# ShudaLi/rgbd_pose_estimation

Measured on AMD Instinct MI355X. Metric: correspondence-residuals/sec, higher is better.
Workload: dtype f32; 1 GPU; configs[1]: 640x480 dense depth, 307200 3D-3D corr, point-to-point GN step (K1 normal eq + host 6x6 solve + SE3 exp) over inlier mask; corr_rank0=307200, global_corr=307200, collective=none, rccl_ranks=0, rccl_verified=False, repeats=1

## Files before the change

### rgbd_pose_estimation_amd/csrc/rpe_host.hpp

```cpp
#pragma once
#include "../../include/rgbd_pose_hip.h"
#include "rpe_kernels.h"
#include "../include/rpe/linalg.hpp"

#include <dlfcn.h>
#include <rccl/rccl.h>

#include <cstdarg>
#include <ctime>
#include <cstdio>
#include <cstdlib>
#include <cmath>
#include <limits>
#include <atomic>
#include <chrono>
#include <condition_variable>
#include <mutex>
#include <string>
#include <vector>
#include <algorithm>
#include <cctype>
#include <sched.h>
#include <unistd.h>
#include <cstring>

struct rpe_context {
  int device = 0;
  hipStream_t stream = nullptr;
  struct { bool active = false; int kind = 0, mode = 0, grid = 0, runs = 0, batches = 0; double thre_3d = 0, cos_thr = 0, cos_nl = 0;
           unsigned long long base = 0, id = 0, slot_token = 0;
           double last_us = 0, wait_us = 2e6;
           bool pend_late = false;
           std::vector<double> seen_pose; std::vector<int> seen_votes;
           bool pending = false; unsigned long long pend_tag = 0; int pend_votes = 0; double pend_pose[7] = {0, 0, 0, 0, 0, 0, 0}; } sess;
  std::recursive_mutex sess_m;
  hipStream_t stream2 = nullptr;
// ... 261 lines not shown
inline rpe::PoseF pose_f(const double* p12) {
  rpe::PoseF T;
  for (int i = 0; i < 9; i++) T.R[i] = (float)p12[i];
  for (int i = 0; i < 3; i++) T.t[i] = (float)p12[9 + i];
  return T;
}
inline int ensure_maps(rpe_context* c, float** maps, int count, size_t* cap, int64_t n) {
  const size_t bytes = (size_t)n * 3 * sizeof(float);
  if (maps[0] && *cap >= bytes) return RPE_OK;
  HIP_TRY(hipStreamSynchronize(c->stream));
  for (int i = 0; i < count; i++) { if (maps[i]) { HIP_TRY(hipFree(maps[i])); maps[i] = nullptr; } }
  *cap = 0;
  for (int i = 0; i < count; i++) HIP_TRY(hipMalloc((void**)&maps[i], bytes));
  *cap = bytes;
  return RPE_OK;
}
int claim_slots(rpe_context* c, int64_t n);
inline void one_level(const rpe_camera& k, const rpe::Camera& f, rpe_camera* kc, rpe::PyramidGeometry* g) {
  *g = rpe::PyramidGeometry{};
  g->levels = 1; g->cam[0] = f; kc[0] = k;
  for (int l = 1; l <= RPE_MAX_LEVELS; l++) g->off[l] = (int64_t)f.width * f.height;
}

void session_end(rpe_context* c);
void session_close(rpe_context* c);
int session_batch(rpe_context* c, int op, const void* staged, int count, size_t bytes, double* totals);
void session_final_masks(rpe_context* c, const void* staged, size_t bytes, const double* pose7, int votes);
bool session_seen(const rpe_context* c, const double* pose7, int* votes);
bool session_matches(const rpe_context* c, int kind, int mode, double thre_3d, double cos_thr, double cos_nl);

template <class Launch>
inline int resident_host_loop(rpe_context* c, Launch launch, int grid, int nacc, int max_rows, int rows_auto, double cost_scale,
                              double* pose12, int max_iter, double tol, int* it_out, double* step_out, double* cost_out, double* weight_out,
                              const char* what, bool clean = false, bool* first_record_finite = nullptr) {
  const unsigned long long base = c->seq;
  auto hand_over = [&](const double* p, unsigned long long tag) {
    if (p) for (int k = 0; k < 12; k++) { unsigned long long w; std::memcpy(&w, &p[k], 8); c->ctl[1 + k] = w; }
    store_fence();
    c->ctl[0] = tag; c->ctl[15] = tag;
    store_fence();
  };
  hand_over(pose12, base + 1);
  rpe::ReduceTarget rt = host_target(c);
  rt.seq = base;
  if (c->hostex) rt.pose_wait_ticks = 1200000000ull;
  if (c->test_pose_wait_s > 0) rt.pose_wait_ticks = (unsigned long long)(c->test_pose_wait_s * 1e8);
  if (c->test_fault_iter >= 1 && c->test_fault_iter <= max_iter) rt.fault_tag = base + (unsigned long long)c->test_fault_iter;
  const int runs = resident_run_shape(grid, nacc, max_rows, rows_auto, &rt);
  rt.h_out = c->h_big;
  rt.clean = clean;
  c->seq = base;
  {
    const hipError_t e = launch(rt, base);
    if (e != hipSuccess) return fail(RPE_ERR_HIP, "resident launch: %s", hipGetErrorString(e));
  }
  int status = RPE_OK, received = 0, it = 0, rc;
  double step = 0, cost = 0, weight = 0;
  double tp = c->loop_prof ? clock_us() : 0;
  for (;;) {
    c->seq = base + (unsigned long long)received + 1;
    double ne[32], d[6];
    double tot[32];
    if ((rc = wait_host_partials(c, runs, nacc, tot, 0, true))) { status = rc; break; }
    if (nacc == 17) expand_p2p17(tot, ne); else { for (int i = 0; i < 32; i++) ne[i] = i < nacc ? tot[i] : 0.0; }
    if (clean && received == 0 && !record_finite(ne, 29)) { status = kResidentDirty; received++; break; }
    if (clean && received == 0 && first_record_finite) *first_record_finite = true;
    if (c->hostex && (rc = rpe_host_exchange_allreduce_f64(c->hostex, ne, 32))) { status = rc; received++; break; }
    received++;
    if (c->loop_prof) { const double t = clock_us(); if (received > 1) { c->prof_wait_us += t - tp; c->prof_steps++; } tp = t; }
    cost = cost_scale * ne[27]; weight = ne[28];
    if (!rpe::solve_normal_eq6(ne, d, rpe::pivot_floor(c->dtype == RPE_F64))) { status = fail(RPE_ERR_DEGENERATE,
        "%s are not positive definite at iteration %d (weight sum %g)", what, it, ne[28]); break; }
    rpe::se3_left_update(d, pose12);
    step = std::sqrt(d[0] * d[0] + d[1] * d[1] + d[2] * d[2] + d[3] * d[3] + d[4] * d[4] + d[5] * d[5]);
    it = received;
    if (step < tol || received == max_iter) break;
    hand_over(pose12, base + (unsigned long long)received + 1);
    if (c->loop_prof) { const double t = clock_us(); c->prof_host_us += t - tp; tp = t; }
  }
  if (status == kResidentLost) hand_over(nullptr, (base + (unsigned long long)received + 2) | rpe::kResidentStopBit);
  else if (received < max_iter) hand_over(nullptr, (base + (unsigned long long)received + 1) | rpe::kResidentStopBit);
  c->seq = base + (unsigned long long)max_iter + 1;
  *it_out = it; *step_out = step; *cost_out = cost; *weight_out = weight;
  if (status == kResidentLost) {
    note_lost_grid(c);
  }
  return status;
}

}
```

### rgbd_pose_estimation_amd/csrc/rpe_normal_eq.hip

```cpp
#include "rpe_residuals.hpp"

namespace rpe {

__global__ void gn_update_probe_kernel(const double* __restrict__ rec, double* __restrict__ pose, double* __restrict__ step_ok,
                                       double rel_floor) {
  __shared__ double s_rec[32];
  __shared__ double s_pose[12];
  if (threadIdx.x < 32) s_rec[threadIdx.x] = rec[threadIdx.x];
  if (threadIdx.x < 12) s_pose[threadIdx.x] = pose[threadIdx.x];
  __syncthreads();
  if (threadIdx.x == 0) {
    double step = 0.0;
    const bool ok = gn_solve_update<0>(s_rec, s_pose, &step, rel_floor);
    step_ok[0] = step; step_ok[1] = ok ? 1.0 : 0.0;
    if (ok) for (int k = 0; k < 12; k++) pose[k] = s_pose[k];
  }
}
hipError_t launch_gn_update_probe(const double* d_rec, double* d_pose, double* d_step_ok, double pivot_floor, hipStream_t s) {
  hipLaunchKernelGGL(gn_update_probe_kernel, dim3(1), dim3(64), 0, s, d_rec, d_pose, d_step_ok, pivot_floor);
  return hipGetLastError();
}

template <class T, int KIND, int BLK, bool MASK, bool WEIGHT, bool CLEAN>
__global__ __launch_bounds__(BLK) void normal_eq_kernel(const T* __restrict__ xw, const T* __restrict__ b, const T* __restrict__ c,
// ... 67 lines not shown
    if (KIND == KIND_P2PLANE) { c0 = nc0; c1 = nc1; c2 = nc2; }
    __builtin_amdgcn_sched_barrier(0);
    pin16(a0); pin16(a1); pin16(a2); pin16(b0); pin16(b1); pin16(b2);
    if (KIND == KIND_P2PLANE) { pin16(c0); pin16(c1); pin16(c2); }
#pragma unroll
    for (int i = 0; i < P; i++) { if (MASK) m[i] = nm[i]; if (WEIGHT) wv[i] = nwv[i]; }
    g = gn;
  }
  if (blockIdx.x == 0 && threadIdx.x == 0 && full * P < n) {
    T vw[3 * P], vb[3 * P], vc[3 * P];
    short lm[P];
    T lwv[P];
    load_group<T>(xw, full, n, vw);
    load_group<T>(b, full, n, vb);
    if (KIND == KIND_P2PLANE) load_group<T>(c, full, n, vc);
    if (MASK) load_scalars<T, short>(mask, full, n, lm, (short)0);
    if (WEIGHT) load_scalars<T, T>(weight, full, n, lwv, T(0));
    pair_group<T, KIND, MASK, WEIGHT, CLEAN, NACC>(pose, vw, vb, vc, lm, lwv, (int)(n - full * P), carry);
    carried = 1;
  }
  if (carried) flush_pairs<T, NACC>(carry, acc);
  RPE_STAMP(1);
  reduce_and_finish<NACC, kNeLd, KIND == KIND_P2P ? 1 : 0, BLK>(acc, fin);
}

template <class T, int KIND, int BLK, bool MASK, bool WEIGHT, int NREG, int AUTO, bool CLEAN>
__global__ __launch_bounds__(BLK) void normal_eq_resident_kernel(const T* __restrict__ xw, const T* __restrict__ b, const T* __restrict__ c,
                             const short* __restrict__ mask, const T* __restrict__ weight, int64_t n,
                             const unsigned long long* __restrict__ ctl, unsigned long long first_tag, int max_iters, Finish fin) {
  constexpr int P = Pk<T>::P;
  constexpr int NACC = KIND == KIND_P2P ? 17 : 29;
  constexpr bool IN_REGS = NREG > 0;
  constexpr int GPT = IN_REGS ? NREG : 1;
  __shared__ double s_pose[12];
  __shared__ int s_go;
  const int64_t full = n / P, groups = (n + P - 1) / P;
  constexpr bool with_solver = AUTO == 2;
  const int workers = (int)gridDim.x;
  const int64_t stride = (int64_t)workers * BLK;
  const int64_t g0 = (int64_t)blockIdx.x * (BLK * GPT) + threadIdx.x;
  T rw[GPT][3 * P], rb[GPT][3 * P], rc[GPT][3 * P];
  short rm[GPT][P];
  T rwv[GPT][P];
  int rpresent[GPT];
#pragma unroll
  for (int r = 0; r < GPT; r++) {
    rpresent[r] = 0;
    const int64_t g = g0 + (int64_t)r * BLK;
    if (IN_REGS && g < groups) {
      load_any_group<T, KIND, MASK, WEIGHT>(xw, b, c, mask, weight, g, full, n, rw[r], rb[r], rc[r], rm[r], rwv[r]);
      rpresent[r] = g < full ? P : (int)(n - full * P);
    }
  }
#ifdef RPE_SOLVER_DEBUG
  if (with_solver && threadIdx.x == 0) __hip_atomic_store(solver_pose_area(fin, workers, NACC) + 32 + blockIdx.x, wall_clock64(), __ATOMIC_RELAXED, __HIP_MEMORY_SCOPE_AGENT);
#endif
  constexpr bool autonomous = AUTO != 0;
  double tol = 0.0;
  if (autonomous) {
    if (threadIdx.x < 12) s_pose[threadIdx.x] = fin.gn_pose[threadIdx.x];
    tol = fin.gn->tol;
    __syncthreads();
  }
  for (int it = 1; it <= max_iters; it++) {
    if (!autonomous && resident_wait_pose<BLK>(ctl, first_tag + (unsigned long long)it, s_pose, &s_go,
        fin.pose_wait_ticks) != 1) return;
    if (with_solver && it > 1 && solver_wait_pose<BLK>(solver_pose_area(fin, workers, NACC), first_tag + (unsigned long long)it, s_pose, &s_go, it == 2 ? kSolverMeetTicks : 200000000ull) != 0) return;
#ifdef RPE_STAMPS
    const bool stamp_it = it == 1000;
    if (stamp_it) RPE_STAMP(0);
#endif
    PoseK<double> pose;
#pragma unroll
    for (int k = 0; k < 9; k++) pose.R[k] = s_pose[k];
#pragma unroll
    for (int k = 0; k < 3; k++) pose.t[k] = s_pose[9 + k];
    double acc[NACC];
#pragma unroll
    for (int k = 0; k < NACC; k++) acc[k] = 0.0;
    if (IN_REGS) {
#pragma unroll
      for (int r = 0; r < GPT; r++)
        if (rpresent[r] > 0) normal_eq_group<T, KIND, MASK, WEIGHT, NACC, CLEAN>(pose, rw[r], rb[r], rc[r], rm[r], rwv[r], rpresent[r], acc);
    } else {
      for (int64_t g = g0; g < groups; g += stride) {
        T vw[3 * P], vb[3 * P], vc[3 * P];
        short mm[P];
        T ww[P];
        load_any_group<T, KIND, MASK, WEIGHT>(xw, b, c, mask, weight, g, full, n, vw, vb, vc, mm, ww);
        normal_eq_group<T, KIND, MASK, WEIGHT, NACC, CLEAN>(pose, vw, vb, vc, mm, ww, g < full ? P : (int)(n - full * P), acc);
      }
    }
#ifdef RPE_STAMPS
    if (stamp_it) RPE_STAMP(1);
#endif
#ifndef RPE_STAMPS
    const bool stamp_it = false;
#endif
    if (with_solver) { solver_send_sums<NACC, BLK>(acc, fin, first_tag + (unsigned long long)it); continue; }
    if (autonomous) {
      if (resident_auto_stage<NACC, BLK>(acc, fin, first_tag + (unsigned long long)it, it, max_iters, tol, s_pose,
          stamp_it) != 0) return;
      continue;
    }
    if (!resident_cross_stage<NACC, BLK>(acc, fin, first_tag + (unsigned long long)it, fin.seq + (unsigned long long)it,
        stamp_it)) return;
  }
}

#ifdef RPE_STAMPS
}
extern "C" int rpe_debug_read_stamps(unsigned long long* out, int nwords) {
  if (nwords > 4096 * 16) nwords = 4096 * 16;
  if (hipDeviceSynchronize() != hipSuccess) return -1;
  if (hipMemcpyFromSymbol(out, HIP_SYMBOL(rpe::g_stamps), (size_t)nwords * 8) != hipSuccess) return -1;
  static unsigned long long zeros[4096 * 16];
  return hipMemcpyToSymbol(HIP_SYMBOL(rpe::g_stamps), zeros, sizeof(zeros)) == hipSuccess ? 0 : -1;
}
namespace rpe {
#endif

template <int MODE>
__global__ __launch_bounds__(64) void chain_finish_kernel(const double* __restrict__ runs, const double* __restrict__ pose_in, GnState* st,
                                                          double rel_floor, double* __restrict__ h_pairs, unsigned long long seq) {
  __shared__ double f_tot[32];
  __shared__ double f_pose[12];
  __shared__ double f_out[16];
  if (threadIdx.x < 12) f_pose[threadIdx.x] = pose_in[threadIdx.x];
  if (threadIdx.x < 32) {
    double t = 0.0;
#pragma unroll
    for (int r = 0; r < kRunSlots; r++) t += runs[r * kRunLd + threadIdx.x];
    f_tot[threadIdx.x] = t;
  }
  __syncthreads();
  if (threadIdx.x == 0) {
    double step = st->step;
    bool ok = st->status == 0;
    if (!st->done) ok = gn_solve_update<MODE>(f_tot, f_pose, &step, rel_floor);
// ... 180 lines not shown
```

### rgbd_pose_estimation_amd/csrc/rpe_reduce.hpp

```cpp
#pragma once
#include "rpe_kernels.h"
#include <cstring>
#include <cstdlib>
#include <algorithm>
#include <hip/hip_ext.h>

namespace rpe {

#ifdef RPE_STAMPS
static __device__ unsigned long long g_stamps[4096 * 16];
#define RPE_STAMP(k)                                                                                             \
  do {                                                                                                           \
    __builtin_amdgcn_sched_barrier(0);                                                                           \
    if (threadIdx.x == 0) {                                                                                      \
      unsigned long long t_;                                                                                     \
      asm volatile("s_memrealtime %0\n\ts_waitcnt lgkmcnt(0)" : "=s"(t_) : : "memory");                          \
      g_stamps[(size_t)blockIdx.x * 16 + (k)] = t_;                                                              \
    }                                                                                                            \
    __builtin_amdgcn_sched_barrier(0);                                                                           \
  } while (0)
#else
#define RPE_STAMP(k) do {} while (0)
#endif

// ... 142 lines not shown
  return __hiloint2double((int)hi[0], (int)lo[0]) + __hiloint2double((int)hi[1], (int)lo[1]);
}
template <int CTRL> __device__ __forceinline__ double pair_add(double x, double y, bool upper) {
  const double keep = upper ? y : x, give = upper ? x : y;
  return keep + dpp_move<CTRL, 0xf>(give);
}
__device__ __forceinline__ double wave_reduce_scatter32(const double (&v)[32], int lane) {
  double a[16], b[8], c[4], d[2];
#pragma unroll
  for (int j = 0; j < 16; j++) a[j] = swap_add32(v[j], v[j + 16]);
#pragma unroll
  for (int j = 0; j < 8; j++) b[j] = swap_add16(a[j], a[j + 8]);
#pragma unroll
  for (int j = 0; j < 4; j++) c[j] = pair_add<0x128>(b[j], b[j + 4], (lane & 8) != 0);
#pragma unroll
  for (int j = 0; j < 2; j++) d[j] = pair_add<0x141>(c[j], c[j + 2], (lane & 4) != 0);
  double e = pair_add<0x1b>(d[0], d[1], (lane & 2) != 0);
  e += dpp_move<0xb1, 0xf>(e);
  return e;
}
__device__ __forceinline__ double wave_reduce_scatter16(const double (&v)[16], int lane) {
  double a[8], b[4], c[2];
#pragma unroll
  for (int j = 0; j < 8; j++) a[j] = swap_add32(v[j], v[j + 8]);
#pragma unroll
  for (int j = 0; j < 4; j++) b[j] = swap_add16(a[j], a[j + 4]);
#pragma unroll
  for (int j = 0; j < 2; j++) c[j] = pair_add<0x128>(b[j], b[j + 2], (lane & 8) != 0);
  double d = pair_add<0x141>(c[0], c[1], (lane & 4) != 0);
  d += dpp_move<0x1b, 0xf>(d);
  d += dpp_move<0xb1, 0xf>(d);
  return d;
}
template <int NACC>
__device__ __forceinline__ void wave_reduce_to(const double (&acc)[NACC], double* __restrict__ out, int lane) {
  int done = 0;
  if constexpr (NACC >= 24) {
    double v[32];
#pragma unroll
    for (int k = 0; k < 32; k++) v[k] = k < NACC ? acc[k] : 0.0;
    const double r = wave_reduce_scatter32(v, lane);
    if ((lane & 1) == 0 && (lane >> 1) < NACC) out[lane >> 1] = r;
    done = 32;
  } else if constexpr (NACC >= 12) {
    double v[16];
#pragma unroll
    for (int k = 0; k < 16; k++) v[k] = acc[k];
    const double r = wave_reduce_scatter16(v, lane);
    if ((lane & 3) == 0) out[(lane >> 2) & 15] = r;
    done = 16;
  }
  if constexpr (NACC > 32 && NACC - 32 > 4) {
    double v[16];
#pragma unroll
    for (int k = 0; k < 16; k++) v[k] = 32 + k < NACC ? acc[32 + k < NACC ? 32 + k : 0] : 0.0;
    const double r = wave_reduce_scatter16(v, lane);
    if ((lane & 3) == 0 && 32 + ((lane >> 2) & 15) < NACC) out[32 + ((lane >> 2) & 15)] = r;
    done = 48;
  }
#pragma unroll
  for (int k = 0; k < NACC; k++) {
    if (k >= done) {
      const double t = wave_sum_to_lane63(acc[k]);
      if (lane == 63) out[k] = t;
    }
  }
}

struct Finish {
  double* partials;
  unsigned int* ticket;
  double* out_dev;
  double* out_host;
  unsigned long long seq;
  double* gn_pose;
  GnState* gn;
  const P2PDesc* p2p;
  unsigned long long p2p_step;
  int tail;
  int rows;
  int stride;
  unsigned long long pose_wait_ticks;
  unsigned long long fault_tag;
// ... 573 lines not shown
```

### rgbd_pose_estimation_amd/csrc/rpe_refine.hip

```cpp
#include "rpe_host.hpp"
#include <memory>
using namespace rpeh;

namespace rpeh {
ResidentSlot& resident_mutex(int device) {
  static ResidentSlot m[64];
  return m[device >= 0 && device < 64 ? device : 0];
}

int resident_run_shape(int grid, int nacc, int max_rows, int rows_auto, rpe::ReduceTarget* rt) {
  static const int env_rows = getenv("RPE_RESIDENT_ROWS") ? atoi(getenv("RPE_RESIDENT_ROWS")) : 0;
  static const int env_stride = run_stride_from_env();
  rt->stride = 0;
  if (env_rows >= 1) rt->rows = std::min(env_rows, max_rows);
  else if (grid * nacc <= 1024) rt->rows = 1;
  else if (env_stride > 1 && grid >= 4 * env_stride && (grid + env_stride - 1) / env_stride <= max_rows) {
    rt->stride = env_stride; rt->rows = (grid + env_stride - 1) / env_stride;
    return env_stride;
  } else rt->rows = rows_auto;
  return (grid + rt->rows - 1) / rt->rows;
}

void note_lost_grid(rpe_context* c) {
  if (++c->resident_lost >= 2) c->resident = false;
// ... 241 lines not shown
  }
  int it = 0;
  double step = 0, cost = 0;
  const double sc = scales ? scales[0] : 1.0;
  const bool sharded_ok = c->hostex ? !c->hostex_shared_gpu : (!c->comm && c->p2p_world_saved < 1);
  if (c->resident && c->host_resident && max_iter >= 2 && sharded_ok && rpe::normal_eq_resident_fits(c->arrays(), kinds[0], c->max_blocks)) {
    int rc = kind_arrays(c, kinds[0]);
    if (rc) return rc;
    if ((rc = check_flags(c, kinds[0], flags))) return rc;
    HIP_TRY(hipSetDevice(c->device));
    if (c->host_cpu_request != -2 && !c->host_cpu_done) {
      c->host_cpu_done = true;
      if (c->host_cpu_request >= 0) (void)pin_calling_thread(c->host_cpu_request);
      else if (!c->hostex && !c->comm && c->p2p_world < 1 && c->p2p_world_saved < 1)
        (void)rpe_tune_host_thread(c, kinds[0], flags, pose12, 200, 5, nullptr, nullptr, nullptr, nullptr, 0, nullptr);
    }
    int grid = 0, nacc = 0, max_rows = 1, rows_auto = 1;
    rpe::resident_geometry(c->arrays(), kinds[0], c->max_blocks, &grid, &nacc, &max_rows, &rows_auto);
    const int kind = kinds[0];
    double weight = 0;
    auto launch = [&](const rpe::ReduceTarget& rt, unsigned long long base) -> hipError_t {
      hipEvent_t e0 = nullptr, e1 = nullptr;
      if (c->timing && c->ev_used < c->ev0.size() && (c->timing_calls++ % c->timing_stride) == 0) { e0 = c->ev0[c->ev_used];
          e1 = c->ev1[c->ev_used]; c->ev_used++; }
      return rpe::launch_normal_eq_resident(c->arrays(), kind, flags, (const unsigned long long*)c->ctl, base, max_iter, rt, c->stream,
          e0, e1);
    };
    for (int attempt = 0; attempt < 2; attempt++) {
      const bool clean = take_clean(c, kind, true);
      bool verified = false;
      { SlotHold one_resident_grid(resident_mutex(c->device));
        if (!one_resident_grid) { rc = kResidentBusy; it = 0; break; }
        rc = resident_host_loop(c, launch, grid, nacc, max_rows, rows_auto, sc, pose12, max_iter, tol, &it, &step, &cost, &weight,
            "normal equations", clean, &verified); }
      if (clean && rc == kResidentDirty) note_clean_launch(c, kind, false);
      else if (clean && verified) note_clean_launch(c, kind, true);
      if (rc != kResidentDirty) break;
      it = 0;
    }
    if (rc != kResidentLost && rc != kResidentBusy) {
      if (iters_out) *iters_out = it;
      if (rc != RPE_OK) return rc;
      if (last_step) *last_step = step;
      if (final_cost) *final_cost = cost;
      return RPE_OK;
    }
  }
  for (; it < max_iter; it++) {
    double ne[32], d[6];
    int rc = rpe_normal_eq(c, kinds[0], flags, pose12, ne);
    if (rc) return rc;
    if (c->hostex && (rc = rpe_host_exchange_allreduce_f64(c->hostex, ne, 32))) return rc;
    cost = sc * ne[27];
    if (!rpe::solve_normal_eq6(ne, d, rpe::pivot_floor(c->dtype == RPE_F64))) {
      if (iters_out) *iters_out = it;
      return fail(RPE_ERR_DEGENERATE, "normal equations are not positive definite at iteration %d (weight sum %g)", it, ne[28]);
    }
    rpe::se3_left_update(d, pose12);
    step = std::sqrt(d[0] * d[0] + d[1] * d[1] + d[2] * d[2] + d[3] * d[3] + d[4] * d[4] + d[5] * d[5]);
    if (step < tol) { it++; break; }
  }
  if (iters_out) *iters_out = it;
  if (last_step) *last_step = step;
  if (final_cost) *final_cost = cost;
  return RPE_OK;
}

// ... 68 lines not shown
```

### rgbd_pose_estimation_amd/csrc/rpe_residuals.hpp

```cpp
#pragma once
#include "rpe_reduce.hpp"

namespace rpe {

template <class C> __device__ __forceinline__ void add_row(const C (&J)[6], C r, C w, C (&s)[29]) {
  int k = 0;
#pragma unroll
  for (int a = 0; a < 6; a++) {
    const C wa = w * J[a];
#pragma unroll
    for (int b = a; b < 6; b++) { s[k] = fma(wa, J[b], s[k]); k++; }
    s[21 + a] = fma(wa, r, s[21 + a]);
  }
  s[27] = fma(w * r, r, s[27]);
}
template <class V> __device__ __forceinline__ void add_row2(const V (&J)[6], V r, V w, V (&s)[29]) {
  int k = 0;
#pragma unroll
  for (int a = 0; a < 6; a++) {
    const V wa = w * J[a];
#pragma unroll
    for (int b = a; b < 6; b++) { s[k] = __builtin_elementwise_fma(wa, J[b], s[k]); k++; }
    s[21 + a] = __builtin_elementwise_fma(wa, r, s[21 + a]);
  }
// ... 144 lines not shown
  typedef C V __attribute__((ext_vector_type(2)));
  const V BX = {bx[0], bx[1]}, BY = {by[0], by[1]}, BZ = {bz[0], bz[1]};
  V e1[3], e2[3];
  tangent_basis<V>(BX, BY, BZ, e1, e2);
  C px[2], py[2], pz[2], d1[2], d2[2];
#pragma unroll
  for (int e = 0; e < 2; e++) {
    double pxd, pyd, pzd;
    transform<C>(T, x[e], y[e], z[e], pxd, pyd, pzd);
    px[e] = (C)pxd; py[e] = (C)pyd; pz[e] = (C)pzd;
    d1[e] = (C)dot_e_p(e1[0][e], e1[1][e], e1[2][e], pxd, pyd, pzd);
    d2[e] = (C)dot_e_p(e2[0][e], e2[1][e], e2[2][e], pxd, pyd, pzd);
  }
  bearing_rows<V>(V{px[0], px[1]}, V{py[0], py[1]}, V{pz[0], pz[1]}, e1, e2, V{d1[0], d1[1]}, V{d2[0], d2[1]}, BX, BY, BZ,
      V{w[0], w[1]},
                  V{w[0], w[1]}, s);
}


template <class V> __device__ __forceinline__ void p2p_accumulate(V px, V py, V pz, V rx, V ry, V rz, V w, V (&s)[17]) {
  const V wpx = w * px, wpy = w * py, wpz = w * pz;
  const V wrx = w * rx, wry = w * ry, wrz = w * rz;
  s[0] += w;
  s[1] += wpx; s[2] += wpy; s[3] += wpz;
  s[4] = __builtin_elementwise_fma(wpx, px, s[4]); s[5] = __builtin_elementwise_fma(wpx, py, s[5]);
  s[6] = __builtin_elementwise_fma(wpx, pz, s[6]); s[7] = __builtin_elementwise_fma(wpy, py, s[7]);
  s[8] = __builtin_elementwise_fma(wpy, pz, s[8]); s[9] = __builtin_elementwise_fma(wpz, pz, s[9]);
  s[10] += wrx; s[11] += wry; s[12] += wrz;
  s[13] += py * wrz - pz * wry;
  s[14] += pz * wrx - px * wrz;
  s[15] += px * wry - py * wrx;
  s[16] = __builtin_elementwise_fma(wrx, rx, __builtin_elementwise_fma(wry, ry, __builtin_elementwise_fma(wrz, rz, s[16])));
}
template <class C>
__device__ __forceinline__ void p2p_pair(const PoseK<double>& T, const C (&x)[2], const C (&y)[2], const C (&z)[2], const C (&cx)[2],
                                         const C (&cy)[2], const C (&cz)[2], const C (&w)[2], C __attribute__((ext_vector_type(2))) (&s)[17]) {
  typedef C V __attribute__((ext_vector_type(2)));
  C px[2], py[2], pz[2], rx[2], ry[2], rz[2];
#pragma unroll
  for (int e = 0; e < 2; e++) {
    double pxd, pyd, pzd;
    transform<C>(T, x[e], y[e], z[e], pxd, pyd, pzd);
    px[e] = (C)pxd; py[e] = (C)pyd; pz[e] = (C)pzd;
    rx[e] = (C)(pxd - (double)cx[e]); ry[e] = (C)(pyd - (double)cy[e]); rz[e] = (C)(pzd - (double)cz[e]);
  }
  p2p_accumulate<V>(V{px[0], px[1]}, V{py[0], py[1]}, V{pz[0], pz[1]}, V{rx[0], rx[1]}, V{ry[0], ry[1]}, V{rz[0], rz[1]}, V{w[0], w[1]}, s);
}

template <class T, int KIND, bool MASK, bool WEIGHT, bool CLEAN, int NS>
__device__ __forceinline__ void pair_group(const PoseK<double>& pose, const T (&vw)[3 * Pk<T>::P], const T (&vb)[3 * Pk<T>::P],
                                           const T (&vc)[3 * Pk<T>::P], const short (&m)[Pk<T>::P], const T (&wv)[Pk<T>::P],
                                           int npresent, T __attribute__((ext_vector_type(2))) (&s2)[NS]) {
  constexpr int P = Pk<T>::P;
  static_assert(NS == (KIND == KIND_P2P ? 17 : 29), "sums per kind");
  static_assert(KIND == KIND_P2P || KIND == KIND_P2PLANE || KIND == KIND_BEARING || KIND == KIND_REPROJ, "residual kinds");
#pragma unroll
  for (int j = 0; j < P / 2; j++) {
    T x[2], y[2], z[2], bx[2], by[2], bz[2], nx[2], ny[2], nz[2], wi[2];
#pragma unroll
    for (int e = 0; e < 2; e++) {
      const int i = 2 * j + e;
      bx[e] = vb[3 * i]; by[e] = vb[3 * i + 1]; bz[e] = vb[3 * i + 2];
      T w = WEIGHT ? wv[i] : T(1);
      if (MASK) w = m[i] == 1 ? w : T(0);
      if (CLEAN) {
        w = i < npresent ? w : T(0);
        x[e] = vw[3 * i]; y[e] = vw[3 * i + 1]; z[e] = vw[3 * i + 2];
        if (KIND == KIND_P2PLANE) { nx[e] = vc[3 * i]; ny[e] = vc[3 * i + 1]; nz[e] = vc[3 * i + 2]; }
      } else {
        w = (i < npresent && !all_nan(bx[e], by[e], bz[e])) ? w : T(0);
        const bool off = w == T(0);
        x[e] = off ? T(0) : vw[3 * i]; y[e] = off ? T(0) : vw[3 * i + 1];
        z[e] = off ? ((KIND == KIND_BEARING || KIND == KIND_REPROJ) ? T(1) : T(0)) : vw[3 * i + 2];
        bx[e] = off ? T(0) : bx[e]; by[e] = off ? T(0) : by[e]; bz[e] = off ? T(1) : bz[e];
        if (KIND == KIND_P2PLANE) { nx[e] = off ? T(0) : vc[3 * i]; ny[e] = off ? T(0) : vc[3 * i + 1];
            nz[e] = off ? T(0) : vc[3 * i + 2]; }
      }
      wi[e] = w;
    }
    if constexpr (KIND == KIND_P2P) p2p_pair<T>(pose, x, y, z, bx, by, bz, wi, s2);
    else if constexpr (KIND == KIND_P2PLANE) p2plane_pair<T>(pose, x, y, z, bx, by, bz, nx, ny, nz, wi, s2);
    else if constexpr (KIND == KIND_BEARING) bearing_pair<T>(pose, x, y, z, bx, by, bz, wi, s2);
    else {
      reproj_pair<T>(pose, x, y, z, bx, by, bz, wi, s2);
      if (CLEAN) {
        typedef T V __attribute__((ext_vector_type(2)));
        const V all = ((V{x[0], x[1]} + V{y[0], y[1]}) + (V{z[0], z[1]} + V{bx[0], bx[1]})) + (V{by[0], by[1]} + V{bz[0], bz[1]});
        s2[27] = __builtin_elementwise_fma(V{T(0), T(0)}, all, s2[27]);
      }
    }
  }
}
template <class T, int NS>
__device__ __forceinline__ void flush_pairs(T __attribute__((ext_vector_type(2))) (&s2)[NS], double (&acc)[NS]) {
  typedef T V __attribute__((ext_vector_type(2)));
#pragma unroll
  for (int k = 0; k < NS; k++) { acc[k] += (double)(s2[k].x + s2[k].y); s2[k] = V{T(0), T(0)}; }
}

template <class T, int KIND, bool MASK, bool WEIGHT, int NACC, bool CLEAN = false>
__device__ __forceinline__ void normal_eq_group(const PoseK<double>& pose, const T (&vw)[3 * Pk<T>::P], const T (&vb)[3 * Pk<T>::P],
                                                const T (&vc)[3 * Pk<T>::P], const short (&m)[Pk<T>::P], const T (&wv)[Pk<T>::P],
                                                int npresent, double (&acc)[NACC]) {
  typedef T V __attribute__((ext_vector_type(2)));
  V s2[NACC];
#pragma unroll
  for (int k = 0; k < NACC; k++) s2[k] = V{T(0), T(0)};
  pair_group<T, KIND, MASK, WEIGHT, CLEAN, NACC>(pose, vw, vb, vc, m, wv, npresent, s2);
  flush_pairs<T, NACC>(s2, acc);
}
constexpr unsigned long long kResidentStop = 1ull << 63;
template <class T, int KIND, bool MASK, bool WEIGHT>
__device__ __forceinline__ void load_any_group(const T* __restrict__ xw, const T* __restrict__ b, const T* __restrict__ c,
                                               const short* __restrict__ mask, const T* __restrict__ weight, int64_t g, int64_t full,
                                               int64_t n, T (&vw)[3 * Pk<T>::P], T (&vb)[3 * Pk<T>::P], T (&vc)[3 * Pk<T>::P],
                                               short (&m)[Pk<T>::P], T (&wv)[Pk<T>::P]) {
  typedef typename Pk<T>::V V;
  if (g < full) {
    const V* xw4 = reinterpret_cast<const V*>(xw);
    const V* b4 = reinterpret_cast<const V*>(b);
    const V x0 = xw4[3 * g], x1 = xw4[3 * g + 1], x2 = xw4[3 * g + 2];
    const V y0 = b4[3 * g], y1 = b4[3 * g + 1], y2 = b4[3 * g + 2];
    unpack3(x0, x1, x2, vw);
    unpack3(y0, y1, y2, vb);
    if (KIND == KIND_P2PLANE) { const V* c4 = reinterpret_cast<const V*>(c);
        const V z0 = c4[3 * g], z1 = c4[3 * g + 1], z2 = c4[3 * g + 2]; unpack3(z0, z1, z2, vc); }
    if (MASK) load_mask_full(mask, g, m);
    if (WEIGHT) load_weight_full(weight, g, wv);
  } else {
    load_group<T>(xw, g, n, vw);
    load_group<T>(b, g, n, vb);
    if (KIND == KIND_P2PLANE) load_group<T>(c, g, n, vc);
    if (MASK) load_scalars<T, short>(mask, g, n, m, (short)0);
    if (WEIGHT) load_scalars<T, T>(weight, g, n, wv, T(0));
  }
}

constexpr int kAutoMaxRunSums = 1024;
__device__ __forceinline__ int resident_judge_pose(unsigned long long w, unsigned long long want) {
  const unsigned int lo = (unsigned int)w, hi = (unsigned int)(w >> 32);
  const unsigned long long ta = ((unsigned long long)__builtin_amdgcn_readlane(hi, 0) << 32) | __builtin_amdgcn_readlane(lo, 0);
  const unsigned long long tb = ((unsigned long long)__builtin_amdgcn_readlane(hi, 15) << 32) | __builtin_amdgcn_readlane(lo, 15);
// ... 56 lines not shown
  if (stamp_it) RPE_STAMP(2);
#endif
  const int rows = rs.rows;
  const bool lost = collect_rows<NACC, BLK>(gran, (int)gridDim.x, leader, rows, tag, g_part, rs.step);
#ifdef RPE_STAMPS
  if (stamp_it) RPE_STAMP(3);
#endif
  const bool ok = !__syncthreads_or(lost);
#ifdef RPE_STAMPS
  if (stamp_it) RPE_STAMP(4);
#endif
  if (threadIdx.x < NACC) store_tagged_pair(fin.out_host, run * NACC + threadIdx.x,
      ok ? sum_rows_lane<NACC, RGN>(g_part, rows < RGN ? rows : RGN, threadIdx.x) : __longlong_as_double((long long)kLostMarker), seq);
#ifdef RPE_STAMPS
  if (stamp_it) RPE_STAMP(5);
#endif
  return ok;
}
template <int NACC, int BLK>
__device__ __forceinline__ bool resident_cross_stage(const double (&acc)[NACC], const Finish& fin, unsigned long long tag,
                                                     unsigned long long seq, bool stamp_it) {
  constexpr int NW = BLK / 64;
  __shared__ double g_red[NW][NACC];
  const int lane = threadIdx.x & 63, wave = threadIdx.x >> 6;
  wave_reduce_to<NACC>(acc, g_red[wave], lane);
  __syncthreads();
  double own = 0.0;
  if (threadIdx.x < NACC) {
#pragma unroll
    for (int w = 0; w < NW; w++) own += g_red[w][threadIdx.x];
  }
  return resident_cross_own<NACC, BLK>(own, fin, tag, seq, stamp_it);
}

template <int NACC, int BLK>
__device__ __forceinline__ int resident_auto_stage(const double (&acc)[NACC], const Finish& fin, unsigned long long tag, int it,
                                                   int max_iters, double tol, double* __restrict__ s_pose, bool stamp_it = false) {
  constexpr int NW = BLK / 64;
  constexpr int RGN = BLK / NACC;
  constexpr int MODE = NACC == 17 ? 1 : 0;
  __shared__ double a_red[NW][NACC];
  __shared__ double a_part[RGN][NACC];
  __shared__ double a_runs[kAutoMaxRunSums];
  __shared__ double a_tot[32];
  __shared__ double a_step;
  __shared__ int a_ok;
  const int lane = threadIdx.x & 63, wave = threadIdx.x >> 6;
  const int G = (int)gridDim.x;
  const RunShape rs = run_shape(fin, G);
  const int run = rs.run, leader = rs.leader, runs = rs.runs;
  unsigned long long* gran = reinterpret_cast<unsigned long long*>(fin.partials);
  unsigned long long* rrec = gran + 2 * ((size_t)G * NACC + (size_t)(it & 1) * runs * NACC);
  wave_reduce_to<NACC>(acc, a_red[wave], lane);
  __syncthreads();
  if (threadIdx.x < NACC) {
    double own = 0.0;
#pragma unroll
    for (int w = 0; w < NW; w++) own += a_red[w][threadIdx.x];
    if ((int)blockIdx.x != leader) store_granule16(gran + 2 * ((size_t)blockIdx.x * NACC + threadIdx.x), own, tag);
    else a_part[0][threadIdx.x] = own;
  }
#ifdef RPE_STAMPS
  if (stamp_it) RPE_STAMP(2);
#endif
  bool lost = runs * NACC > kAutoMaxRunSums;
  if (!lost && (int)blockIdx.x == leader) {
// ... 206 lines not shown
```

Before: 48.15 billion correspondence-residuals/s.

## Hoist pose-independent point moments out of resident point-to-point GN loop

For point-to-point normal equations in the resident host-driven kernel, the pose-independent weighted moments of the source points (sum w, sum w·x, sum w·xxᵀ) are computed once before the iteration loop. Each iteration then accumulates and reduces only the 7 residual-dependent sums instead of 17. The host rebuilds the full 17-entry record from the moments and the current pose. This cuts per-iteration FLOPs, reduction width and host/device transfer. It adds a one-time extra pass, and the moment-to-sum transform may lose some precision for large translations.

```diff
diff --git a/rgbd_pose_estimation_amd/csrc/rpe_host.hpp b/rgbd_pose_estimation_amd/csrc/rpe_host.hpp
--- a/rgbd_pose_estimation_amd/csrc/rpe_host.hpp
+++ b/rgbd_pose_estimation_amd/csrc/rpe_host.hpp
@@ -2,6 +2,7 @@
 #include "../../include/rgbd_pose_hip.h"
 #include "rpe_kernels.h"
 #include "../include/rpe/linalg.hpp"
+#include "../include/rpe/p2p_moments.hpp"
 
 #include <dlfcn.h>
 #include <rccl/rccl.h>
@@ -329,8 +330,9 @@
 template <class Launch>
 inline int resident_host_loop(rpe_context* c, Launch launch, int grid, int nacc, int max_rows, int rows_auto, double cost_scale,
                               double* pose12, int max_iter, double tol, int* it_out, double* step_out, double* cost_out, double* weight_out,
-                              const char* what, bool clean = false, bool* first_record_finite = nullptr) {
+                              const char* what, bool clean = false, bool* first_record_finite = nullptr, bool p2p_moments = false) {
   const unsigned long long base = c->seq;
+  double mom[10] = {0, 0, 0, 0, 0, 0, 0, 0, 0, 0};
   auto hand_over = [&](const double* p, unsigned long long tag) {
     if (p) for (int k = 0; k < 12; k++) { unsigned long long w; std::memcpy(&w, &p[k], 8); c->ctl[1 + k] = w; }
     store_fence();
@@ -358,7 +360,12 @@
     c->seq = base + (unsigned long long)received + 1;
     double ne[32], d[6];
     double tot[32];
-    if ((rc = wait_host_partials(c, runs, nacc, tot, 0, true))) { status = rc; break; }
+    if ((rc = wait_host_partials(c, runs, p2p_moments && received > 0 ? 7 : nacc, tot, 0, true))) { status = rc; break; }
+    if (p2p_moments) {
+      if (received == 0) std::memcpy(mom, tot, sizeof(mom));
+      else for (int k = 0; k < 7; k++) tot[10 + k] = tot[k];
+      rpe::p2p_sums_from_moments(mom, pose12, tot);
+    }
     if (nacc == 17) expand_p2p17(tot, ne); else { for (int i = 0; i < 32; i++) ne[i] = i < nacc ? tot[i] : 0.0; }
     if (clean && received == 0 && !record_finite(ne, 29)) { status = kResidentDirty; received++; break; }
     if (clean && received == 0 && first_record_finite) *first_record_finite = true;
diff --git a/rgbd_pose_estimation_amd/csrc/rpe_normal_eq.hip b/rgbd_pose_estimation_amd/csrc/rpe_normal_eq.hip
--- a/rgbd_pose_estimation_amd/csrc/rpe_normal_eq.hip
+++ b/rgbd_pose_estimation_amd/csrc/rpe_normal_eq.hip
@@ -123,6 +123,9 @@
   constexpr int NACC = KIND == KIND_P2P ? 17 : 29;
   constexpr bool IN_REGS = NREG > 0;
   constexpr int GPT = IN_REGS ? NREG : 1;
+  constexpr bool HOIST = KIND == KIND_P2P && AUTO == 0;
+  constexpr int NSUM = HOIST ? 7 : NACC;
+  __shared__ double s_mom[HOIST ? BLK / 64 : 1][10];
   __shared__ double s_pose[12];
   __shared__ int s_go;
   const int64_t full = n / P, groups = (n + P - 1) / P;
@@ -147,6 +150,30 @@
   if (with_solver && threadIdx.x == 0) __hip_atomic_store(solver_pose_area(fin, workers, NACC) + 32 + blockIdx.x, wall_clock64(), __ATOMIC_RELAXED, __HIP_MEMORY_SCOPE_AGENT);
 #endif
   constexpr bool autonomous = AUTO != 0;
+  if constexpr (HOIST) {
+    double mom[10];
+#pragma unroll
+    for (int k = 0; k < 10; k++) mom[k] = 0.0;
+    if (IN_REGS) {
+#pragma unroll
+      for (int r = 0; r < GPT; r++)
+        if (rpresent[r] > 0) p2p_moments_group<T, MASK, WEIGHT, CLEAN>(rw[r], rb[r], rm[r], rwv[r], rpresent[r], mom);
+    } else {
+      for (int64_t g = g0; g < groups; g += stride) {
+        T vw[3 * P], vb[3 * P], vc[3 * P];
+        short mm[P];
+        T ww[P];
+        load_any_group<T, KIND, MASK, WEIGHT>(xw, b, c, mask, weight, g, full, n, vw, vb, vc, mm, ww);
+        p2p_moments_group<T, MASK, WEIGHT, CLEAN>(vw, vb, mm, ww, g < full ? P : (int)(n - full * P), mom);
+      }
+    }
+    double v[16];
+#pragma unroll
+    for (int k = 0; k < 16; k++) v[k] = k < 10 ? mom[k < 10 ? k : 0] : 0.0;
+    const int lane = threadIdx.x & 63;
+    const double tot = wave_reduce_scatter16(v, lane);
+    if ((lane & 3) == 0 && ((lane >> 2) & 15) < 10) s_mom[threadIdx.x >> 6][(lane >> 2) & 15] = tot;
+  }
   double tol = 0.0;
   if (autonomous) {
     if (threadIdx.x < 12) s_pose[threadIdx.x] = fin.gn_pose[threadIdx.x];
@@ -166,20 +193,20 @@
     for (int k = 0; k < 9; k++) pose.R[k] = s_pose[k];
 #pragma unroll
     for (int k = 0; k < 3; k++) pose.t[k] = s_pose[9 + k];
-    double acc[NACC];
-#pragma unroll
-    for (int k = 0; k < NACC; k++) acc[k] = 0.0;
+    double acc[NSUM];
+#pragma unroll
+    for (int k = 0; k < NSUM; k++) acc[k] = 0.0;
     if (IN_REGS) {
 #pragma unroll
       for (int r = 0; r < GPT; r++)
-        if (rpresent[r] > 0) normal_eq_group<T, KIND, MASK, WEIGHT, NACC, CLEAN>(pose, rw[r], rb[r], rc[r], rm[r], rwv[r], rpresent[r], acc);
+        if (rpresent[r] > 0) normal_eq_group<T, KIND, MASK, WEIGHT, NSUM, CLEAN>(pose, rw[r], rb[r], rc[r], rm[r], rwv[r], rpresent[r], acc);
     } else {
       for (int64_t g = g0; g < groups; g += stride) {
         T vw[3 * P], vb[3 * P], vc[3 * P];
         short mm[P];
         T ww[P];
         load_any_group<T, KIND, MASK, WEIGHT>(xw, b, c, mask, weight, g, full, n, vw, vb, vc, mm, ww);
-        normal_eq_group<T, KIND, MASK, WEIGHT, NACC, CLEAN>(pose, vw, vb, vc, mm, ww, g < full ? P : (int)(n - full * P), acc);
+        normal_eq_group<T, KIND, MASK, WEIGHT, NSUM, CLEAN>(pose, vw, vb, vc, mm, ww, g < full ? P : (int)(n - full * P), acc);
       }
     }
 #ifdef RPE_STAMPS
@@ -188,14 +215,19 @@
 #ifndef RPE_STAMPS
     const bool stamp_it = false;
 #endif
-    if (with_solver) { solver_send_sums<NACC, BLK>(acc, fin, first_tag + (unsigned long long)it); continue; }
-    if (autonomous) {
-      if (resident_auto_stage<NACC, BLK>(acc, fin, first_tag + (unsigned long long)it, it, max_iters, tol, s_pose,
-          stamp_it) != 0) return;
-      continue;
+    if constexpr (HOIST) {
+      if (!resident_cross_stage_p2p_hoisted<BLK>(acc, s_mom, it == 1, fin, first_tag + (unsigned long long)it,
+          fin.seq + (unsigned long long)it, stamp_it)) return;
+    } else {
+      if (with_solver) { solver_send_sums<NACC, BLK>(acc, fin, first_tag + (unsigned long long)it); continue; }
+      if (autonomous) {
+        if (resident_auto_stage<NACC, BLK>(acc, fin, first_tag + (unsigned long long)it, it, max_iters, tol, s_pose,
+            stamp_it) != 0) return;
+        continue;
+      }
+      if (!resident_cross_stage<NACC, BLK>(acc, fin, first_tag + (unsigned long long)it, fin.seq + (unsigned long long)it,
+          stamp_it)) return;
     }
-    if (!resident_cross_stage<NACC, BLK>(acc, fin, first_tag + (unsigned long long)it, fin.seq + (unsigned long long)it,
-        stamp_it)) return;
   }
 }
 
diff --git a/rgbd_pose_estimation_amd/csrc/rpe_reduce.hpp b/rgbd_pose_estimation_amd/csrc/rpe_reduce.hpp
--- a/rgbd_pose_estimation_amd/csrc/rpe_reduce.hpp
+++ b/rgbd_pose_estimation_amd/csrc/rpe_reduce.hpp
@@ -198,6 +198,18 @@
   d += dpp_move<0xb1, 0xf>(d);
   return d;
 }
+__device__ __forceinline__ double wave_reduce_scatter8(const double (&v)[8], int lane) {
+  double a[4], b[2];
+#pragma unroll
+  for (int j = 0; j < 4; j++) a[j] = swap_add32(v[j], v[j + 4]);
+#pragma unroll
+  for (int j = 0; j < 2; j++) b[j] = swap_add16(a[j], a[j + 2]);
+  double c = pair_add<0x128>(b[0], b[1], (lane & 8) != 0);
+  c += dpp_move<0x141, 0xf>(c);
+  c += dpp_move<0x1b, 0xf>(c);
+  c += dpp_move<0xb1, 0xf>(c);
+  return c;
+}
 template <int NACC>
 __device__ __forceinline__ void wave_reduce_to(const double (&acc)[NACC], double* __restrict__ out, int lane) {
   int done = 0;
@@ -215,6 +227,13 @@
     const double r = wave_reduce_scatter16(v, lane);
     if ((lane & 3) == 0) out[(lane >> 2) & 15] = r;
     done = 16;
+  } else if constexpr (NACC == 7) {
+    double v[8];
+#pragma unroll
+    for (int k = 0; k < 8; k++) v[k] = k < NACC ? acc[k < NACC ? k : 0] : 0.0;
+    const double r = wave_reduce_scatter8(v, lane);
+    if ((lane & 7) == 0 && ((lane >> 3) & 7) < NACC) out[(lane >> 3) & 7] = r;
+    done = 8;
   }
   if constexpr (NACC > 32 && NACC - 32 > 4) {
     double v[16];
diff --git a/rgbd_pose_estimation_amd/csrc/rpe_refine.hip b/rgbd_pose_estimation_amd/csrc/rpe_refine.hip
--- a/rgbd_pose_estimation_amd/csrc/rpe_refine.hip
+++ b/rgbd_pose_estimation_amd/csrc/rpe_refine.hip
@@ -297,7 +297,7 @@
       { SlotHold one_resident_grid(resident_mutex(c->device));
         if (!one_resident_grid) { rc = kResidentBusy; it = 0; break; }
         rc = resident_host_loop(c, launch, grid, nacc, max_rows, rows_auto, sc, pose12, max_iter, tol, &it, &step, &cost, &weight,
-            "normal equations", clean, &verified); }
+            "normal equations", clean, &verified, kind == RPE_RES_P2P); }
       if (clean && rc == kResidentDirty) note_clean_launch(c, kind, false);
       else if (clean && verified) note_clean_launch(c, kind, true);
       if (rc != kResidentDirty) break;
diff --git a/rgbd_pose_estimation_amd/csrc/rpe_residuals.hpp b/rgbd_pose_estimation_amd/csrc/rpe_residuals.hpp
--- a/rgbd_pose_estimation_amd/csrc/rpe_residuals.hpp
+++ b/rgbd_pose_estimation_amd/csrc/rpe_residuals.hpp
@@ -200,9 +200,17 @@
   s[15] += px * wry - py * wrx;
   s[16] = __builtin_elementwise_fma(wrx, rx, __builtin_elementwise_fma(wry, ry, __builtin_elementwise_fma(wrz, rz, s[16])));
 }
-template <class C>
+template <class V> __device__ __forceinline__ void p2p_accumulate(V px, V py, V pz, V rx, V ry, V rz, V w, V (&s)[7]) {
+  const V wrx = w * rx, wry = w * ry, wrz = w * rz;
+  s[0] += wrx; s[1] += wry; s[2] += wrz;
+  s[3] += py * wrz - pz * wry;
+  s[4] += pz * wrx - px * wrz;
+  s[5] += px * wry - py * wrx;
+  s[6] = __builtin_elementwise_fma(wrx, rx, __builtin_elementwise_fma(wry, ry, __builtin_elementwise_fma(wrz, rz, s[6])));
+}
+template <class C, int NS>
 __device__ __forceinline__ void p2p_pair(const PoseK<double>& T, const C (&x)[2], const C (&y)[2], const C (&z)[2], const C (&cx)[2],
-                                         const C (&cy)[2], const C (&cz)[2], const C (&w)[2], C __attribute__((ext_vector_type(2))) (&s)[17]) {
+                                         const C (&cy)[2], const C (&cz)[2], const C (&w)[2], C __attribute__((ext_vector_type(2))) (&s)[NS]) {
   typedef C V __attribute__((ext_vector_type(2)));
   C px[2], py[2], pz[2], rx[2], ry[2], rz[2];
 #pragma unroll
@@ -220,7 +228,7 @@
                                            const T (&vc)[3 * Pk<T>::P], const short (&m)[Pk<T>::P], const T (&wv)[Pk<T>::P],
                                            int npresent, T __attribute__((ext_vector_type(2))) (&s2)[NS]) {
   constexpr int P = Pk<T>::P;
-  static_assert(NS == (KIND == KIND_P2P ? 17 : 29), "sums per kind");
+  static_assert(NS == (KIND == KIND_P2P ? 17 : 29) || (KIND == KIND_P2P && NS == 7), "sums per kind (point-to-point: 7 = the residual sums alone)");
   static_assert(KIND == KIND_P2P || KIND == KIND_P2PLANE || KIND == KIND_BEARING || KIND == KIND_REPROJ, "residual kinds");
 #pragma unroll
   for (int j = 0; j < P / 2; j++) {
@@ -246,7 +254,7 @@
       }
       wi[e] = w;
     }
-    if constexpr (KIND == KIND_P2P) p2p_pair<T>(pose, x, y, z, bx, by, bz, wi, s2);
+    if constexpr (KIND == KIND_P2P) p2p_pair<T, NS>(pose, x, y, z, bx, by, bz, wi, s2);
     else if constexpr (KIND == KIND_P2PLANE) p2plane_pair<T>(pose, x, y, z, bx, by, bz, nx, ny, nz, wi, s2);
     else if constexpr (KIND == KIND_BEARING) bearing_pair<T>(pose, x, y, z, bx, by, bz, wi, s2);
     else {
@@ -276,6 +284,29 @@
   for (int k = 0; k < NACC; k++) s2[k] = V{T(0), T(0)};
   pair_group<T, KIND, MASK, WEIGHT, CLEAN, NACC>(pose, vw, vb, vc, m, wv, npresent, s2);
   flush_pairs<T, NACC>(s2, acc);
+}
+template <class T, bool MASK, bool WEIGHT, bool CLEAN>
+__device__ __forceinline__ void p2p_moments_group(const T (&vw)[3 * Pk<T>::P], const T (&vb)[3 * Pk<T>::P], const short (&m)[Pk<T>::P],
+                                                  const T (&wv)[Pk<T>::P], int npresent, double (&mom)[10]) {
+  constexpr int P = Pk<T>::P;
+#pragma unroll
+  for (int i = 0; i < P; i++) {
+    T w = WEIGHT ? wv[i] : T(1);
+    if (MASK) w = m[i] == 1 ? w : T(0);
+    T x = vw[3 * i], y = vw[3 * i + 1], z = vw[3 * i + 2];
+    if (CLEAN) w = i < npresent ? w : T(0);
+    else {
+      w = (i < npresent && !all_nan(vb[3 * i], vb[3 * i + 1], vb[3 * i + 2])) ? w : T(0);
+      const bool off = w == T(0);
+      x = off ? T(0) : x; y = off ? T(0) : y; z = off ? T(0) : z;
+    }
+    const double wd = w, xd = x, yd = y, zd = z;
+    const double wx = wd * xd, wy = wd * yd, wz = wd * zd;
+    mom[0] += wd;
+    mom[1] += wx; mom[2] += wy; mom[3] += wz;
+    mom[4] = fma(wx, xd, mom[4]); mom[5] = fma(wx, yd, mom[5]); mom[6] = fma(wx, zd, mom[6]);
+    mom[7] = fma(wy, yd, mom[7]); mom[8] = fma(wy, zd, mom[8]); mom[9] = fma(wz, zd, mom[9]);
+  }
 }
 constexpr unsigned long long kResidentStop = 1ull << 63;
 template <class T, int KIND, bool MASK, bool WEIGHT>
@@ -398,6 +429,32 @@
   }
   return resident_cross_own<NACC, BLK>(own, fin, tag, seq, stamp_it);
 }
+template <int BLK>
+__device__ __forceinline__ bool resident_cross_stage_p2p_hoisted(const double (&acc)[7], const double (*s_mom)[10], bool first,
+                                                                 const Finish& fin, unsigned long long tag, unsigned long long seq,
+                                                                 bool stamp_it) {
+  constexpr int NW = BLK / 64;
+  __shared__ double h_red[NW][7];
+  const int lane = threadIdx.x & 63, wave = threadIdx.x >> 6;
+  wave_reduce_to<7>(acc, h_red[wave], lane);
+  __syncthreads();
+  double own = 0.0;
+  if (first) {
+    if (threadIdx.x < 10) {
+#pragma unroll
+      for (int w = 0; w < NW; w++) own += s_mom[w][threadIdx.x];
+    } else if (threadIdx.x < 17) {
+#pragma unroll
+      for (int w = 0; w < NW; w++) own += h_red[w][threadIdx.x - 10];
+    }
+    return resident_cross_own<17, BLK>(own, fin, tag, seq, stamp_it);
+  }
+  if (threadIdx.x < 7) {
+#pragma unroll
+    for (int w = 0; w < NW; w++) own += h_red[w][threadIdx.x];
+  }
+  return resident_cross_own<7, BLK>(own, fin, tag, seq, stamp_it);
+}
 
 template <int NACC, int BLK>
 __device__ __forceinline__ int resident_auto_stage(const double (&acc)[NACC], const Finish& fin, unsigned long long tag, int it,
diff --git a/rgbd_pose_estimation_amd/include/rpe/p2p_moments.hpp b/rgbd_pose_estimation_amd/include/rpe/p2p_moments.hpp
--- /dev/null
+++ b/rgbd_pose_estimation_amd/include/rpe/p2p_moments.hpp
@@ -0,0 +1,26 @@
+#pragma once
+
+namespace rpe {
+
+inline void p2p_sums_from_moments(const double mom[10], const double pose12[12], double out[10]) {
+  const double* R = pose12;
+  const double* t = pose12 + 9;
+  const double m0 = mom[0];
+  const double M2[3][3] = {{mom[4], mom[5], mom[6]}, {mom[5], mom[7], mom[8]}, {mom[6], mom[8], mom[9]}};
+  double a[3];
+  double RM[3][3];
+  for (int i = 0; i < 3; i++) {
+    a[i] = R[3 * i] * mom[1] + R[3 * i + 1] * mom[2] + R[3 * i + 2] * mom[3];
+    for (int j = 0; j < 3; j++) RM[i][j] = R[3 * i] * M2[0][j] + R[3 * i + 1] * M2[1][j] + R[3 * i + 2] * M2[2][j];
+  }
+  out[0] = m0;
+  for (int i = 0; i < 3; i++) out[1 + i] = a[i] + t[i] * m0;
+  int k = 4;
+  for (int i = 0; i < 3; i++)
+    for (int j = i; j < 3; j++) {
+      const double rmr = RM[i][0] * R[3 * j] + RM[i][1] * R[3 * j + 1] + RM[i][2] * R[3 * j + 2];
+      out[k++] = rmr + a[i] * t[j] + t[i] * a[j] + m0 * t[i] * t[j];
+    }
+}
+
+}
```

New measurement: 50.87 billion correspondence-residuals/s, median of 4. 5.6% higher.
